# JuliaRobotics/IncrementalInference.jl

Hardware: AMD Instinct MI355X
Metric: clique-messages/sec (higher is better)
Workload: dtype f64; 1 GPU; config 2: ContinuousEuclid(2) 1000-variable odometry chain + priors every 100, N=200 particles, nested-dissection order, full up+down solveTree; variables_per_gpu=1000, particles=200, cliques=983, parallelism=single GPU

## Files before the change

include/nbp.h:

```cpp
#ifndef NBP_H
#define NBP_H

#include <stdint.h>

#ifdef __cplusplus
extern "C" {
#endif

#define NBP_MAXV 6
#define NBP_MAXF 128
#define NBP_MAXD 3
#define NBP_MAXC 4
#define NBP_MAXK 8
#define NBP_MAXN 512
#define NBP_COMP_STRIDE 13
enum nbp_dist {
  NBP_DIST_GAUSSIAN = 0,
  NBP_DIST_UNIFORM = 1,
  NBP_DIST_RAYLEIGH = 2,
  NBP_DIST_TABLE = 3
};

typedef int32_t nbp_status;
#define NBP_OK 0
// ... 326 lines not shown
  NBP_STAGE_COPIES = 3,
  NBP_STAGE_DECONV = 4,
  NBP_STAGE_COPY_POINTS = 5
};
nbp_status nbp_program_create(nbp_ctx *ctx, nbp_program **out);
nbp_status nbp_program_add_stage(nbp_program *prog, int32_t kind, const void *descs, int32_t n);
enum nbp_program_option { NBP_OPT_LAZY_BANDWIDTH = 1, NBP_OPT_GRAPH_REPLAY = 2, NBP_OPT_FUSED_UPDATES = 3,
                          NBP_OPT_ASYNC_UPLOAD = 4  };
nbp_status nbp_program_set_option(nbp_program *prog, int32_t option, int32_t value);
nbp_status nbp_program_finalize(nbp_program *prog);
nbp_status nbp_program_run(nbp_program *prog, int32_t first_stage, int32_t last_stage );
nbp_status nbp_program_reseed(nbp_program *prog, uint64_t salt);
nbp_status nbp_program_num_seeds(nbp_program *prog, int32_t *out);
nbp_status nbp_program_set_seeds(nbp_program *prog, const uint64_t *seeds, int32_t n);
nbp_status nbp_program_seed_order(nbp_program *prog, int32_t *order, int32_t n);
nbp_status nbp_program_num_stages(nbp_program *prog, int32_t *out);
nbp_status nbp_program_num_fused(nbp_program *prog, int32_t *out);
nbp_status nbp_program_num_two_stream(nbp_program *prog, int32_t *out);
nbp_status nbp_program_set_lanes(nbp_program *prog, int32_t stage, const int32_t *lane_of_descriptor, int32_t n);
typedef struct nbp_lane_part_rec {
  int32_t stage, lane, first_desc, n, wait, signals;
} nbp_lane_part_rec;
nbp_status nbp_program_lane_plan(nbp_program *prog, nbp_lane_part_rec *out, int32_t cap, int32_t *n_out);
nbp_status nbp_program_destroy(nbp_program *prog);
nbp_status nbp_program_retire(nbp_program *prog);

#define NBP_COMM_ID_BYTES 128
typedef struct nbp_comm nbp_comm;
#ifndef NBP_XFER_DEFINED
#define NBP_XFER_DEFINED
typedef struct nbp_xfer { int32_t peer; int32_t slot; } nbp_xfer;
#endif
nbp_status nbp_comm_unique_id(void *id_out );
nbp_status nbp_comm_create(nbp_ctx *ctx, int32_t world, int32_t rank, const void *id, nbp_comm **out);
nbp_status nbp_comm_destroy(nbp_comm *comm);
nbp_status nbp_comm_info(nbp_comm *comm, int32_t *nranks_out, int32_t *rank_out);
nbp_status nbp_exchange(nbp_ctx *ctx, nbp_comm *comm, const nbp_xfer *sends, int32_t n_sends, const nbp_xfer *recvs, int32_t n_recvs);

nbp_status nbp_timing_enable(nbp_ctx *ctx, int32_t on);
nbp_status nbp_timing_read(nbp_ctx *ctx, double *ms, int64_t *launches);
nbp_status nbp_timing_read_n(nbp_ctx *ctx, double *ms, int64_t *launches, int32_t n);
nbp_status nbp_diag_read(nbp_ctx *ctx, nbp_diag *out, int32_t reset);

typedef struct nbp_product_plan_req {
  int32_t N;
  int32_t n;
// ... 60 lines not shown
```

include/nbp_host.h:

```cpp
#ifndef NBP_HOST_H
#define NBP_HOST_H
#include "nbp.h"

#ifdef __cplusplus
extern "C" {
#endif

typedef struct nbp_graph nbp_graph;
typedef struct nbp_tree nbp_tree;

typedef struct nbp_solver_params {
  int32_t N;
  int32_t gibbs_iters;
  int32_t inflate_cycles;
  int32_t product_niter;
  int32_t upsolve, downsolve, limitfixeddown;
  int32_t flags;
  double spread_nh;
  double inflation;
  double null_surplus_add;
} nbp_solver_params;

enum nbp_solver_flag {
  NBP_SOLVER_STORED_MEASUREMENTS = 1,
// ... 122 lines not shown
  const nbp_solver_params *params;
  const nbp_clique_desc *clique;
  uint64_t seed;
  nbp_tree_belief *beliefs;
  nbp_tree_belief *diff_out;
  int32_t down;
  int32_t status;
} nbp_clique_request;
nbp_status nbp_clique_solve_batch(nbp_ctx *ctx, nbp_clique_request *requests, int32_t n);

typedef struct nbp_clique_ticket nbp_clique_ticket;
nbp_status nbp_clique_submit_batch(nbp_ctx *ctx, nbp_clique_request *requests, int32_t n, nbp_clique_ticket **ticket_out);
nbp_status nbp_clique_wait(nbp_clique_ticket *ticket);
nbp_status nbp_resident_write(nbp_ctx *ctx, int32_t n, const int32_t *handles, const int32_t *manifolds, const nbp_tree_belief *beliefs);
nbp_status nbp_resident_read(nbp_ctx *ctx, int32_t n, const int32_t *handles, const int32_t *manifolds, nbp_tree_belief *beliefs);
nbp_status nbp_resident_copy(nbp_ctx *ctx, int32_t n, const int32_t *src_handles, const int32_t *dst_handles, int32_t points_only);

nbp_status nbp_clique_seam_times(double *seconds_out6, int32_t mode);

int32_t nbp_tree_num_stages(const nbp_tree *t);
nbp_status nbp_tree_stage(const nbp_tree *t, int32_t s, int32_t *kind, int32_t *n, void *descs_out, int64_t cap_bytes);
nbp_status nbp_tree_stage_lanes(const nbp_tree *t, int32_t s, int32_t *lanes_out, int32_t cap);
nbp_status nbp_tree_stage_promoted(const nbp_tree *t, int32_t s, int32_t *promoted_out, int32_t cap);

#ifdef __cplusplus
}
#endif
#endif
```

incrementalinference.jl_amd/abi.py:

```python
import ctypes as C
import os

MAXV, MAXF, MAXD, MAXC, MAXN, COMP_STRIDE = 6, 128, 3, 4, 512, 13

EUCLID1, EUCLID2, EUCLID3, CIRCULAR, SE2 = 1, 2, 3, 4, 5
F_PRIOR, F_MSGPRIOR, F_LINREL, F_CIRCULAR, F_SE2, F_EUCLIDDIST, F_PASSTHROUGH = 1, 2, 3, 4, 5, 6, 7
DIST_GAUSSIAN, DIST_UNIFORM, DIST_RAYLEIGH, DIST_TABLE = 0, 1, 2, 3
STAGE_PROPOSALS, STAGE_PRODUCTS, STAGE_COPIES, STAGE_DECONV, STAGE_COPY_POINTS = 1, 2, 3, 4, 5
OPT_LAZY_BANDWIDTH = 1
OPT_GRAPH_REPLAY = 2
OPT_FUSED_UPDATES = 3

MANIFOLD_DIM = {EUCLID1: 1, EUCLID2: 2, EUCLID3: 3, CIRCULAR: 1, SE2: 3}
MANIFOLD_P = {EUCLID1: 1, EUCLID2: 2, EUCLID3: 3, CIRCULAR: 1, SE2: 6}


class ProposalDesc(C.Structure):
    _fields_ = [
        ("factor_kind", C.c_int32),
        ("manifold", C.c_int32),
        ("nvars", C.c_int32),
        ("sfidx", C.c_int32),
        ("var_slot", C.c_int32 * MAXV),
        ("out_slot", C.c_int32),
# ... 204 lines not shown
def plan_fits(reqs):
    return _plan("nbp_plan_fits", FitPlanReq, FitPlanRec, reqs)


def plan_proposals(reqs):
    return _plan("nbp_plan_proposals", ProposalPlanReq, ProposalPlanRec, reqs)


def slot_stride(N):
    return 3 * N + 8


_PKG_DIR = os.path.dirname(os.path.abspath(__file__))
LIB_PATH = os.path.join(_PKG_DIR, "csrc", "libnbp.so")

EXPORTS = [
    "nbp_arena_bytes", "nbp_slot_stride_doubles", "nbp_ctx_create", "nbp_ctx_destroy",
    "nbp_last_error", "nbp_synchronize", "nbp_arena_ptr", "nbp_stream_ptr", "nbp_ctx_particles", "nbp_ctx_slots", "nbp_ctx_device",
    "nbp_ctx_reserve_resident", "nbp_ctx_resident", "nbp_belief_write_batch_async", "nbp_belief_read_batch_begin", "nbp_belief_read_batch_end",
    "nbp_run_copies_async", "nbp_program_retire",
    "nbp_slot_write", "nbp_slot_read", "nbp_belief_write", "nbp_belief_read", "nbp_belief_write_batch", "nbp_belief_read_batch", "nbp_run_resample", "nbp_side_write", "nbp_side_read",
    "nbp_run_proposals", "nbp_run_bandwidth", "nbp_run_ppe", "nbp_kde_ppe", "nbp_run_evaluate", "nbp_kde_evaluate", "nbp_run_marginal_grid", "nbp_kde_marginal_grid", "nbp_run_evaluate_marginal", "nbp_run_mmd", "nbp_kde_mmd", "nbp_run_meancov", "nbp_kde_meancov", "nbp_run_kld", "nbp_kde_kld", "nbp_run_overlap", "nbp_kde_overlap", "nbp_run_overlap_search", "nbp_run_scene_grid", "nbp_run_credible", "nbp_kde_credible", "nbp_run_modes", "nbp_kde_modes", "nbp_run_mixture", "nbp_kde_mixture", "nbp_run_factor_likelihood", "nbp_factor_likelihood", "nbp_run_factor_mode_likelihood", "nbp_factor_mode_likelihood", "nbp_heatmap_create", "nbp_heatmap_build", "nbp_heatmap_draw", "nbp_heatmap_info", "nbp_heatmap_destroy", "nbp_heatmap_scan_eval", "nbp_heatmap_search_eval", "nbp_run_products", "nbp_run_copies", "nbp_run_deconv", "nbp_kde_bandwidth", "nbp_conv", "nbp_manifold_product",
    "nbp_program_create", "nbp_program_add_stage", "nbp_program_set_option", "nbp_program_finalize", "nbp_program_run",
    "nbp_program_reseed", "nbp_program_num_seeds", "nbp_program_set_seeds", "nbp_program_seed_order", "nbp_ctx_attach", "nbp_ctx_attached", "nbp_program_num_stages", "nbp_program_num_fused", "nbp_program_num_two_stream", "nbp_program_set_lanes", "nbp_program_lane_plan", "nbp_program_destroy",
    "nbp_timing_enable", "nbp_timing_read", "nbp_timing_read_n", "nbp_diag_read",
    "nbp_plan_products", "nbp_plan_fits", "nbp_plan_proposals", "nbp_last_plans",
    "nbp_comm_unique_id", "nbp_comm_create", "nbp_comm_destroy", "nbp_comm_info", "nbp_exchange", "nbp_math_eval",
]

_lib = None


def load_library(path=None):
    global _lib
    if _lib is not None and path is None:
        return _lib
    path = path or os.environ.get("NBP_LIB_OVERRIDE") or LIB_PATH
    if not os.path.exists(path):
        raise RuntimeError(
            f"libnbp.so not found at {path}: build it with `python __graft_entry__.py` "
            "(hipcc --offload-arch=gfx950). The product path has no CPU fallback."
        )
    try:
        import torch
    except ImportError:
        pass
    lib = C.CDLL(path)
# ... 72 lines not shown
    lib.nbp_program_add_stage.argtypes = [vp, i32, vp, i32]
    lib.nbp_program_set_option.argtypes = [vp, i32, i32]
    lib.nbp_program_finalize.argtypes = [vp]
    lib.nbp_program_run.argtypes = [vp, i32, i32]
    lib.nbp_program_reseed.argtypes = [vp, C.c_uint64]
    lib.nbp_program_num_seeds.argtypes = [vp, ip]
    lib.nbp_program_set_seeds.argtypes = [vp, C.POINTER(C.c_uint64), i32]
    lib.nbp_program_seed_order.argtypes = [vp, ip, i32]
    lib.nbp_program_num_stages.argtypes = [vp, ip]
    lib.nbp_program_destroy.argtypes = [vp]
    lib.nbp_comm_unique_id.argtypes = [vp]
    lib.nbp_comm_create.argtypes = [vp, i32, i32, vp, C.POINTER(vp)]
    lib.nbp_comm_destroy.argtypes = [vp]
    lib.nbp_comm_info.argtypes = [vp, ip, ip]
    lib.nbp_math_eval.argtypes = [vp, i32, dp, dp, dp, dp, i64]
    lib.nbp_exchange.argtypes = [vp, vp, C.POINTER(Xfer), i32, C.POINTER(Xfer), i32]
    lib.nbp_timing_enable.argtypes = [vp, i32]
    lib.nbp_timing_read.argtypes = [vp, dp, C.POINTER(i64)]
    lib.nbp_timing_read_n.argtypes = [vp, dp, C.POINTER(i64), i32]
    lib.nbp_program_num_fused.argtypes = [vp, C.POINTER(i32)]
    lib.nbp_program_num_two_stream.argtypes = [vp, C.POINTER(i32)]
    lib.nbp_program_set_lanes.argtypes = [vp, i32, ip, i32]
    lib.nbp_program_lane_plan.argtypes = [vp, C.POINTER(LanePartRec), i32, C.POINTER(i32)]
    lib.nbp_diag_read.argtypes = [vp, C.POINTER(Diag), i32]
    lib.nbp_plan_products.argtypes = [C.POINTER(ProductPlanReq), C.POINTER(ProductPlanRec), i64]
    lib.nbp_plan_fits.argtypes = [C.POINTER(FitPlanReq), C.POINTER(FitPlanRec), i64]
    lib.nbp_plan_proposals.argtypes = [C.POINTER(ProposalPlanReq), C.POINTER(ProposalPlanRec), i64]
    lib.nbp_last_plans.argtypes = [vp, C.POINTER(ProductPlanRec), C.POINTER(FitPlanRec), C.POINTER(FitPlanRec)]
    for name in EXPORTS:
        fn = getattr(lib, name)
        if fn.restype is C.c_int:
            fn.restype = C.c_int32
    if path == LIB_PATH:
        _lib = lib
    return lib
```

incrementalinference.jl_amd/backend.py:

```python
import ctypes as C
import weakref

import numpy as np

from . import abi


class NbpError(RuntimeError):
    """Hard error from libnbp (status < 0).  The Julia shim maps this to `error()`, which fails
    the clique Task and makes `monitorCSMs` tear the solve down with a CompositeException
    (reference: CliqStateMachineUtils.jl:184-246, test/testCSMMonitor.jl:51)."""


_IP, _DP = C.POINTER(C.c_int32), C.POINTER(C.c_double)


def _i32(seq):
    a = np.ascontiguousarray(seq, dtype=np.int32)
    return a, a.ctypes.data_as(_IP)


def _f64(a, shape=None):
    a = np.ascontiguousarray(a, dtype=np.float64)
    a = a if shape is None else a.reshape(shape)
# ... 662 lines not shown
        self._p = C.c_void_p()
        backend._check(lib.nbp_program_create(backend._ctx, C.byref(self._p)))
        backend._programs.add(self)
        if lazy_bandwidth:
            backend._check(lib.nbp_program_set_option(self._p, abi.OPT_LAZY_BANDWIDTH, 1))
        if not fused_updates:
            backend._check(lib.nbp_program_set_option(self._p, abi.OPT_FUSED_UPDATES, 0))
        for kind, descs in stages:
            arr, n = _as_array(descs, _STAGE_CTYPE[kind])
            backend._check(lib.nbp_program_add_stage(self._p, kind, C.cast(arr, C.c_void_p), n))
        for s, hint in (lanes or {}).items():
            arr = (C.c_int32 * max(len(hint), 1))(*[int(x) for x in hint])
            backend._check(lib.nbp_program_set_lanes(self._p, s, arr, len(hint)))
        backend._check(lib.nbp_program_finalize(self._p))
        self.n_stages = len(stages)

    def lane_plan(self):
        n = C.c_int32(0)
        self.backend._check(self.backend.lib.nbp_program_lane_plan(self._p, None, 0, C.byref(n)))
        recs = (abi.LanePartRec * max(n.value, 1))()
        self.backend._check(self.backend.lib.nbp_program_lane_plan(self._p, recs, n.value, C.byref(n)))
        return [{k: getattr(r, k) for k, _ in abi.LanePartRec._fields_} for r in recs[:n.value]]

    def num_fused(self):
        n = C.c_int32(0)
        self.backend._check(self.backend.lib.nbp_program_num_fused(self._p, C.byref(n)))
        return n.value

    def num_two_stream(self):
        n = C.c_int32(0)
        self.backend._check(self.backend.lib.nbp_program_num_two_stream(self._p, C.byref(n)))
        return n.value

    def run(self, first=0, last=-1):
        self.backend._check(self.backend.lib.nbp_program_run(self._p, first, last))

    def reseed(self, salt):
        self.backend._check(self.backend.lib.nbp_program_reseed(self._p, C.c_uint64(salt)))

    def num_seeds(self):
        n = C.c_int32(0)
        self.backend._check(self.backend.lib.nbp_program_num_seeds(self._p, C.byref(n)))
        return n.value

    def set_seeds(self, seeds):
        arr = (C.c_uint64 * len(seeds))(*[int(x) for x in seeds])
# ... 32 lines not shown
```

incrementalinference.jl_amd/csrc/nbp_api.hip:

```cpp
#include <hip/hip_runtime.h>

#include <cmath>
#include <cstdio>
#include <cstring>
#include <string>
#include <thread>
#include <vector>

#include <unordered_map>

#include <dlfcn.h>
#include <algorithm>
#include <rccl/rccl.h>

#ifndef NBP_TU
#define NBP_TU 0
#endif
#include "nbp_kernels.h"
#include "nbp_fused.h"
#include "nbp_ppe.h"
#include "nbp_query.h"
#include "nbp_stats.h"
#include "nbp_marginal.h"
#include "nbp_heatmap.h"
// ... 2578 lines not shown
  NBPCHK(stage_columns(c, {{slots, 4 * (size_t)n}, {manifolds, 4 * (size_t)n}}, d, 0));
  NBPCHK(launch_checked(c, nbp_resample_kernel, n, 256, 0, d[0], d[1], c->arena, c->N, c->S, seed));
  HIPCHK(hipStreamSynchronize(c->stream));
  return NBP_OK;
}

struct nbp_stage {
  int kind = 0, n = 0, maxfd = 0, mani = 0;
  size_t offset = 0;
  nbp_fits ent;
  bool flush_before = false;
  bool need_prep = true;
  bool fused = false, fused_second = false;
  int upd_F = 0;
  std::vector<nbp_update_desc> upd;
  size_t upd_off = 0;
  nbp_fits split_out;
  bool pipe = false;
  int pipe_split = -1, pipe_ent = 0;
  std::vector<int> moved_to;
  std::vector<int32_t> lane_hint;
  int lane_split = -1;
  int lane = 0, user = -1;
  nbp_fits bound;
  std::vector<int> waits;
  bool signals = false;
};
struct nbp_program {
  nbp_ctx *ctx = nullptr;
  std::vector<nbp_stage> stages;
  std::vector<char> blob;
  char *dev = nullptr;
  size_t dev_bytes = 0;
  bool finalized = false;
  bool lazy_bw = false;
  bool use_graph = true;
  bool use_fused = true;
  bool async_upload = false;
  int n_user_stages = 0;
  struct captured { hipGraphExec_t exec; uint64_t ws_gen; };
  std::unordered_map<uint64_t, captured> graphs;
  std::unordered_map<uint64_t, int> runs;
  size_t seed_off = 0;
  size_t seed_val_off = 0;
  int n_seeds = 0;
  std::vector<int32_t> seed_rank;
// ... 446 lines not shown
      if (n == 0 && (l || st.lane_split >= 0)) continue;
      nbp_stage pt;
      pt.kind = st.kind; pt.n = n; pt.offset = st.offset + (size_t)from * esz; pt.lane = l; pt.user = s;
      pt.maxfd = st.maxfd; pt.mani = st.mani;
      if (st.kind == NBP_STAGE_PRODUCTS && st.lane_split >= 0) {
        pt.maxfd = products_maxfd((const nbp_product_desc *)(p->blob.data() + pt.offset), n);
        pt.mani = products_uniform_manifold((const nbp_product_desc *)(p->blob.data() + pt.offset), n);
      }
      if (st.kind == NBP_STAGE_PROPOSALS && st.lane_split >= 0) pt.mani = proposals_uniform_class((const nbp_proposal_desc *)(p->blob.data() + pt.offset), n);
      const std::vector<char> &row = st.kind == NBP_STAGE_PRODUCTS ? live.dead_product[(size_t)s] : live.dead_proposal[(size_t)s];
      dead.push_back(row.empty() ? nullptr : row.data() + from);
      parts.push_back(std::move(pt));
    }
  }
  p->first_part[(size_t)p->n_user_stages] = (int)parts.size();
  {
    nbp_stage pt;
    pt.user = p->n_user_stages;
    dead.push_back(nullptr);
    parts.push_back(std::move(pt));
  }
  nbp_fits pend[2];
  std::vector<nbp_fits> ran(parts.size());
  for (int k = 0; k < (int)parts.size(); k++) {
    nbp_stage &st = parts[(size_t)k];
    const int l = st.lane, o = 1 - l;
    const char *d = p->blob.data() + st.offset;
    if (k == p->first_part[(size_t)st.user]) {
      st.bound = pend[0];
      for (const nbp_fits::fit &f : pend[1].v) st.bound.push(f.slot, f.mani);
    }
    if (st.kind == NBP_STAGE_DECONV || st.kind == NBP_STAGE_COPY_POINTS)
      stage_writes(p, st, [&](int, int32_t slot) { pend[0].drop(slot); pend[1].drop(slot); });
    if (!pend[o].empty()) {
      auto claim = [&](int32_t slot) {
        for (size_t i = 0; i < pend[o].v.size();)
          if (pend[o].v[i].slot == slot) { pend[l].v.push_back(pend[o].v[i]); pend[o].v.erase(pend[o].v.begin() + (long)i); } else i++;
      };
      stage_reads(p, st, [&](int, int32_t slot, nbp_access a) { if (a != NBP_RD_POINTS || st.kind == NBP_STAGE_PRODUCTS) claim(slot); });
      if (st.kind == NBP_STAGE_PROPOSALS || st.kind == NBP_STAGE_PRODUCTS) stage_writes(p, st, [&](int, int32_t slot) { claim(slot); });
      if (st.kind == NBP_STAGE_COPIES || st.kind == 0) {
        for (const nbp_fits::fit &f : pend[o].v) pend[l].v.push_back(f);
        pend[o].clear();
      }
    }
    st.ent = pend[l];
    auto flush_if_read = [&](nbp_access what) {
      stage_reads(p, st, [&](int, int32_t slot, nbp_access a) { st.flush_before |= a == what && pend[l].has(slot); });
      if (st.flush_before) { for (const nbp_fits::fit &f : pend[l].v) ran[(size_t)k].push(f.slot, f.mani); pend[l].clear(); }
    };
    if (st.kind == NBP_STAGE_PROPOSALS) {
      flush_if_read(NBP_RD_KDE);
      queue_fits(pend[l], (const nbp_proposal_desc *)d, st.n, dead[(size_t)k]);
    } else if (st.kind == NBP_STAGE_PRODUCTS) {
      const nbp_product_desc *qd = (const nbp_product_desc *)d;
      st.need_prep = false;
      for (int i = 0; i < st.n; i++) st.need_prep |= qd[i].nfactors > 1;
      flush_if_read(NBP_RD_POINTS);
      if (st.need_prep) {
        for (const nbp_fits::fit &f : pend[l].v) ran[(size_t)k].push(f.slot, f.mani);
        pend[l].clear();
      } else {
        for (int i = 0; i < st.n; i++) pend[l].rename(qd[i].in_slot[0], qd[i].out_slot);
        pend[l].dedup();
      }
      queue_fits(pend[l], qd, st.n, dead[(size_t)k]);
    } else if (st.kind == NBP_STAGE_DECONV || st.kind == NBP_STAGE_COPY_POINTS) {
      if (st.kind == NBP_STAGE_DECONV)
        for (int i = 0; i < st.n; i++) pend[l].push(((const nbp_proposal_desc *)d)[i].out_slot, ((const nbp_proposal_desc *)d)[i].manifold);
    } else {
      st.flush_before = true;
      for (const nbp_fits::fit &f : pend[l].v) ran[(size_t)k].push(f.slot, f.mani);
      pend[l].clear();
    }
  }
  std::vector<nbp_lane_part> sw(parts.size());
  for (int k = 0; k < (int)parts.size(); k++) {
    const nbp_stage &st = parts[(size_t)k];
    nbp_lane_part &a = sw[(size_t)k];
    a.stage = st.user;
    a.lane = st.lane;
    a.barrier = st.kind == 0 || ((st.kind == NBP_STAGE_COPIES || st.kind == NBP_STAGE_COPY_POINTS) && st.n == 0);
    stage_reads(p, st, [&](int, int32_t slot, nbp_access acc) {
      a.reads.push_back(2 * slot);
      if (acc != NBP_RD_POINTS || st.kind == NBP_STAGE_PRODUCTS) a.reads.push_back(2 * slot + 1);
      if (acc == NBP_RD_POINTS && st.kind == NBP_STAGE_PRODUCTS) a.writes.push_back(2 * slot);
    }, true);
    stage_writes(p, st, [&](int, int32_t slot) {
      a.writes.push_back(2 * slot);
      if (st.kind != NBP_STAGE_COPY_POINTS) a.writes.push_back(2 * slot + 1);
    });
    for (const nbp_fits::fit &f : ran[(size_t)k].v) { a.reads.push_back(2 * f.slot); a.writes.push_back(2 * f.slot + 1); }
    const char *d = p->blob.data() + st.offset;
    for (int i = 0; i < st.n; i++)
      if (st.kind == NBP_STAGE_PROPOSALS || st.kind == NBP_STAGE_DECONV) {
        const nbp_proposal_desc &q = ((const nbp_proposal_desc *)d)[i];
        if (q.mhidx_in >= 0) a.reads.push_back(NBP_LANE_SLOT_SIDE);
        if (q.mhidx_out >= 0) a.writes.push_back(NBP_LANE_SLOT_SIDE);
      } else if (st.kind == NBP_STAGE_PRODUCTS && ((const nbp_product_desc *)d)[i].labels_out >= 0) {
        a.writes.push_back(NBP_LANE_SLOT_SIDE);
      }
  }
  nbp_lane_sweep(sw);
  for (int k = 0; k < (int)parts.size(); k++) {
    parts[(size_t)k].waits = sw[(size_t)k].waits;
// ... 395 lines not shown
nbp_status nbp_program_num_two_stream(nbp_program *p, int32_t *out) {
  if (!p || !out) return fail(NBP_ERR_ARG, "null argument");
  int n = 0;
  for (const nbp_stage &st : p->stages) n += st.pipe ? 1 : 0;
  *out = n;
  return NBP_OK;
}

nbp_status nbp_program_lane_plan(nbp_program *p, nbp_lane_part_rec *out, int32_t cap, int32_t *n_out) {
  if (!p || !n_out || (!out && cap > 0)) return fail(NBP_ERR_ARG, "null argument");
  if (!p->finalized) return fail(NBP_ERR_ARG, "program not finalized");
  const int np = p->parts.empty() ? 0 : (int)p->parts.size() - 1;
  *n_out = np;
  for (int k = 0; k < np && k < cap; k++) {
    const nbp_stage &st = p->parts[(size_t)k];
    const nbp_stage &us = p->stages[(size_t)st.user];
    const size_t esz = st.kind == NBP_STAGE_PRODUCTS ? sizeof(nbp_product_desc) : (st.kind == NBP_STAGE_COPIES || st.kind == NBP_STAGE_COPY_POINTS ?
                       sizeof(nbp_copy_desc) : sizeof(nbp_proposal_desc));
    out[k] = {st.user, st.lane, (int32_t)((st.offset - us.offset) / esz), st.n, st.waits.empty() ? -1 : st.waits[0], st.signals ? 1 : 0};
  }
  return NBP_OK;
}

static void program_free(nbp_program *p, bool sync);
static void reap_retired(nbp_ctx *c) {
  for (size_t i = 0; i < c->retired.size();) {
    if (hipEventQuery(c->retired[i].second) == hipSuccess) {
      hipEventDestroy(c->retired[i].second);
      nbp_program *p = c->retired[i].first;
      c->retired.erase(c->retired.begin() + (long)i);
      program_free(p, false);
    } else
      i++;
  }
}
nbp_status nbp_program_retire(nbp_program *p) {
  if (!p) return NBP_OK;
  if (!p->ctx) { delete p; return NBP_OK; }
  nbp_ctx *c = p->ctx;
  hipSetDevice(c->device);
  reap_retired(c);
  hipEvent_t ev = nullptr;
  if (hipEventCreateWithFlags(&ev, hipEventDisableTiming) != hipSuccess || hipEventRecord(ev, c->stream) != hipSuccess) {
    if (ev) hipEventDestroy(ev);
    return nbp_program_destroy(p);
  }
// ... 370 lines not shown
```

incrementalinference.jl_amd/csrc/nbp_host.cpp:

```cpp
#include <algorithm>
#include <atomic>
#include <chrono>
#include <array>
#include <deque>
#include <cstdio>
#include <cstdlib>
#include <cstring>
#include <map>
#include <set>
#include <string>
#include <condition_variable>
#include <functional>
#include <mutex>
#include <thread>
#include <vector>

#include "../../include/nbp_host.h"

extern "C" nbp_status nbp_internal_fail(nbp_status code, const char *msg);
static nbp_status hfail(nbp_status c, const char *m) { return nbp_internal_fail(c, m); }

namespace {

struct HVar { int manifold; bool initialized, ismargin; };
// ... 1162 lines not shown
    for (const Clique &c : t->cl) {
      if (!(start[c.id] <= tt && tt < finish[c.id]) || !t->mine(c.id)) continue;
      const std::vector<int> &round = (down ? t->drounds : t->urounds)[c.id - 1][tt - start[c.id]];
      for (size_t lane = 0; lane < round.size(); lane++) {
        const int k = round[lane], v = (down ? t->dsched : t->usched)[c.id - 1][k];
        const bool fresh = down || !t->stored || t->uiter[c.id - 1][k] == 1;
        if (nbp_status rc = tree_update(t, c, v, down ? down_entries(t, c, v) : up_entries(t, c, v), down ? PASS_DOWN : PASS_UP, k, seed, props,
                                        prods, fresh, (int)lane))
          return rc;
      }
      plane.resize(props.size(), side.empty() ? 0 : side[c.id]);
      qlane.resize(prods.size(), side.empty() ? 0 : side[c.id]);
    }
    if (!prods.empty()) {
      add_update_stages(t->stages, props, prods);
      if (!side.empty()) {
        t->stages[t->stages.size() - 2].lane = plane;
        t->stages[t->stages.size() - 1].lane = qlane;
      }
    }
    return (nbp_status)NBP_OK;
  };
  const long round_updates = 200;
  auto stragglers = [&](bool down, int T, const std::vector<int> &start, const std::vector<int> &finish) {
    std::vector<char> side;
    if (!t->owner.empty() || T <= 0) return side;
    const int narrow_max = getenv("NBP_LANE_NARROW_MAX") ? atoi(getenv("NBP_LANE_NARROW_MAX")) : 32;
    const bool promote = down && !(getenv("NBP_LANE_NO_PROMOTE") && atoi(getenv("NBP_LANE_NO_PROMOTE")) != 0);
    const auto &rounds = down ? t->drounds : t->urounds;
    std::vector<int> count((size_t)T, 0), held((size_t)T, 0);
    for (const Clique &c : t->cl)
      for (int tt = start[c.id]; tt < finish[c.id]; tt++) count[(size_t)tt] += (int)rounds[c.id - 1][(size_t)(tt - start[c.id])].size();
    side.assign(t->cl.size() + 1, 0);
    bool any = false;
    for (const Clique &c : t->cl) {
      bool narrow = false, wide = false;
      for (int tt = start[c.id]; tt < finish[c.id]; tt++) {
        if (count[(size_t)tt] <= narrow_max) narrow = true; else wide = true;
      }
      if (!(narrow && wide)) continue;
      side[c.id] = 1;
      any = true;
      for (int tt = start[c.id]; tt < finish[c.id]; tt++) held[(size_t)tt] += (int)rounds[c.id - 1][(size_t)(tt - start[c.id])].size();
    }
    if (!any || *std::max_element(held.begin(), held.end()) > 64) side.clear();
    if (side.empty() || !promote) return side;
    std::vector<char> chain(side);
    for (const Clique &c : t->cl) {
      if (!side[c.id]) continue;
      long ahead = 0;
      for (int tt = start[c.id]; tt < T; tt++)
        if (count[(size_t)tt] > narrow_max) ahead += count[(size_t)tt];
      if ((long)(finish[c.id] - start[c.id]) * round_updates <= ahead) continue;
      for (int a = c.parent; a != 0 && !chain[a]; a = t->cl[a - 1].parent) {
        bool wide = false;
        for (int tt = start[a]; tt < finish[a]; tt++) wide |= count[(size_t)tt] > narrow_max;
        if (!wide) break;
        chain[a] = 2;
        for (int tt = start[a]; tt < finish[a]; tt++) held[(size_t)tt] += (int)rounds[a - 1][(size_t)(tt - start[a])].size();
      }
    }
    return *std::max_element(held.begin(), held.end()) > 64 ? side : chain;
  };
  if (g->sp.upsolve) {
    const size_t nc = t->cl.size();
    const std::vector<int> ids = cliques_by(height);
    std::vector<int> start(nc + 1, 0), finish(nc + 1, 0);
    int T = 0;
    for (int cid : ids) {
      int st = 0;
      for (int chd : t->cl[cid - 1].children) st = std::max(st, finish[chd]);
      start[cid] = st;
      finish[cid] = st + (int)t->urounds[cid - 1].size();
      T = std::max(T, finish[cid]);
    }
    const std::vector<char> side = stragglers(false, T, start, finish);
    for (int tt = 0; tt < T; tt++) {
      if (t->joint) {
        props.clear();
        for (const Clique &c : t->cl) {
          if (finish[c.id] != tt || c.parent == 0 || !t->mine(c.id)) continue;
          for (size_t i = 0; i < c.rel.size(); i++)
            props.push_back(deconv_op(g->sp, seed, c.id, (int)i, c.rel[i][3], c.rel[i][0], c.rel[i][1], g->vars[c.rel[i][0]].manifold,
                                      g->vars[c.rel[i][1]].manifold, {&t->B[c.id - 1], &t->main_slot}, c.Dslot[i]));
        }
// ... 16 lines not shown
  };
  cps.clear();
  if (!g->sp.downsolve) {
    for (const Clique &c : t->cl) frontals_out(c, cps);
    add_stage(t->stages, NBP_STAGE_COPIES, cps.data(), sizeof(nbp_copy_desc), (int)cps.size());
  } else {
    for (int r : t->roots) frontals_out(t->cl[r - 1], cps);
    add_stage(t->stages, NBP_STAGE_COPIES, cps.data(), sizeof(nbp_copy_desc), (int)cps.size());
    std::vector<nbp_copy_desc> final_cps;
    for (int dpt = 1; dpt <= maxd; dpt++)
      for (const Clique &c : t->cl)
        if (depth[c.id] == dpt) frontals_out(c, final_cps);
    {
      const size_t nc = t->cl.size();
      const std::vector<int> ids = cliques_by(depth);
      std::vector<int> start(nc + 1, 0), finish(nc + 1, 0);
      int T = 0;
      for (int cid : ids) {
        const Clique &c = t->cl[cid - 1];
        start[cid] = c.parent ? finish[c.parent] : 0;
        finish[cid] = start[cid] + (int)t->drounds[cid - 1].size();
        T = std::max(T, finish[cid]);
      }
      const std::vector<char> side = stragglers(true, T, start, finish);
      for (int tt = 0; tt <= T; tt++) {
        std::map<int, int> rnd;
        int nrounds = 0;
        for (int cid : ids) {
          const Clique &c = t->cl[cid - 1];
          if (start[cid] != tt || !c.parent) continue;
          auto it = rnd.find(c.parent);
          rnd[cid] = it == rnd.end() ? 0 : it->second + 1;
          nrounds = std::max(nrounds, rnd[cid] + 1);
        }
        for (int r = 0; r < nrounds; r++) {
          std::vector<Edge> edges;
          for (const Clique &c : t->cl) {
            auto it = rnd.find(c.id);
            if (it == rnd.end() || it->second != r || t->own(c.id) == t->own(c.parent)) continue;
            for (int s : c.seps)
              edges.push_back({t->own(c.parent), t->mine(c.parent) ? t->B[c.parent - 1].at(s) : -1, t->own(c.id),
                               t->mine(c.id) ? t->B[c.id - 1].at(s) : -1});
          }
          rank_exchange(t, edges);
          cps.clear();
          std::vector<int32_t> clane;
          for (const Clique &c : t->cl) {
// ... 1146 lines not shown
  if (mode >= 1) g_seam_sync.store(mode == 2);
  return NBP_OK;
}

int32_t nbp_tree_num_stages(const nbp_tree *t) { return t ? (int32_t)t->stages.size() : 0; }
nbp_status nbp_tree_stage(const nbp_tree *t, int32_t s, int32_t *kind, int32_t *n, void *out, int64_t cap) {
  if (!t || s < 0 || s >= (int)t->stages.size()) return hfail(NBP_ERR_RANGE, "stage index");
  return stage_out(t->stages[s], kind, n, out, cap);
}
nbp_status nbp_tree_stage_lanes(const nbp_tree *t, int32_t s, int32_t *lanes_out, int32_t cap) {
  if (!t || s < 0 || s >= (int)t->stages.size()) return hfail(NBP_ERR_RANGE, "stage index");
  if (!lanes_out && cap > 0) return hfail(NBP_ERR_ARG, "null argument");
  const Stage &st = t->stages[s];
  for (int i = 0; i < st.n && i < cap; i++) lanes_out[i] = !st.lane.empty() && st.lane[(size_t)i] == 1;
  return NBP_OK;
}
nbp_status nbp_tree_stage_promoted(const nbp_tree *t, int32_t s, int32_t *promoted_out, int32_t cap) {
  if (!t || s < 0 || s >= (int)t->stages.size()) return hfail(NBP_ERR_RANGE, "stage index");
  if (!promoted_out && cap > 0) return hfail(NBP_ERR_ARG, "null argument");
  const Stage &st = t->stages[s];
  for (int i = 0; i < st.n && i < cap; i++) promoted_out[i] = !st.lane.empty() && st.lane[(size_t)i] == 2;
  return NBP_OK;
}

}
```

incrementalinference.jl_amd/native_host.py:

```python
import ctypes as C

import numpy as np

from . import abi

i32, i64, f64 = C.c_int32, C.c_int64, C.c_double


SOLVER_STORED_MEASUREMENTS, SOLVER_MSG_LIKELIHOODS = 1, 2


class SolverParamsC(C.Structure):
    _fields_ = [("N", i32), ("gibbs_iters", i32), ("inflate_cycles", i32), ("product_niter", i32), ("upsolve", i32),
                ("downsolve", i32), ("limitfixeddown", i32), ("flags", i32), ("spread_nh", f64), ("inflation", f64),
                ("null_surplus_add", f64)]


class FactorSpec(C.Structure):
    _fields_ = [("factor_kind", i32), ("nvars", i32), ("vars", i32 * abi.MAXV), ("ncomp", i32), ("has_multihypo", i32),
                ("partial_mask", i32), ("multihypo", f64 * abi.MAXV), ("nullhypo", f64), ("inflation", f64),
                ("comp", (f64 * abi.COMP_STRIDE) * abi.MAXC)]


class CliqueInfo(C.Structure):
# ... 12 lines not shown
class TreeBeliefC(C.Structure):
    _fields_ = [("pts", C.POINTER(f64)), ("bw", C.POINTER(f64)), ("ipc", C.POINTER(f64)), ("n_pts", i32), ("handle", i32)]


class CliqueDescC(C.Structure):
    _fields_ = [("clique_id", i32), ("nvars", i32), ("nfrontals", i32), ("nseparators", i32),
                ("manifold", C.POINTER(i32)), ("ismargin", C.POINTER(i32)), ("nfactors", i32), ("factors", C.POINTER(FactorSpec)),
                ("n_direct_frtl_msg", i32), ("n_msgskip", i32), ("n_itervar", i32), ("n_direct_prior_msg", i32),
                ("direct_frtl_msg", C.POINTER(i32)), ("msgskip", C.POINTER(i32)), ("itervar", C.POINTER(i32)),
                ("direct_prior_msg", C.POINTER(i32)), ("nmsgs", i32), ("msg_var", C.POINTER(i32)),
                ("msg_belief", C.POINTER(TreeBeliefC)), ("factor_density", C.POINTER(TreeBeliefC)),
                ("factor_meas_kde", C.POINTER(TreeBeliefC)), ("n_diff", i32), ("reserved_", i32),
                ("diff_a", C.POINTER(i32)), ("diff_b", C.POINTER(i32)), ("diff_kind", C.POINTER(i32))]


CLIQ_UPSOLVED, CLIQ_DOWNSOLVED = 3, 5
CLIQ_NULL, CLIQ_MARGINALIZED, CLIQ_UPRECYCLED = 0, 4, 6

HOST_EXPORTS = ["nbp_graph_create", "nbp_graph_destroy", "nbp_graph_add_variable", "nbp_graph_add_factor",
                "nbp_graph_set_variable_flags", "nbp_graph_num_variables", "nbp_graph_num_factors",
                "nbp_graph_order_nested_dissection", "nbp_graph_init_plan", "nbp_graph_init_num_variables", "nbp_graph_init_variables",
                "nbp_graph_init_num_stages", "nbp_graph_init_stage", "nbp_graph_init_compile", "nbp_tree_build", "nbp_tree_destroy", "nbp_tree_num_cliques",
                "nbp_tree_clique", "nbp_tree_clique_idlists", "nbp_tree_max_schedule", "nbp_tree_plan_slots", "nbp_tree_main_slots", "nbp_tree_compile", "nbp_tree_schedule",
                "nbp_tree_get_stats", "nbp_tree_num_stages", "nbp_tree_stage", "nbp_tree_stage_lanes", "nbp_tree_stage_promoted", "nbp_clique_slots", "nbp_clique_upsolve", "nbp_clique_upsolve_joint", "nbp_clique_downsolve", "nbp_clique_solve_batch", "nbp_clique_seam_times",
                "nbp_clique_submit_batch", "nbp_clique_wait", "nbp_resident_write", "nbp_resident_read", "nbp_resident_copy",
                "nbp_tree_partition", "nbp_tree_set_owner", "nbp_tree_num_segments", "nbp_tree_segment",
                "nbp_tree_run_sharded", "nbp_tree_run_sharded_cb",
                "nbp_graph_num_densities", "nbp_graph_density_factors", "nbp_graph_init_density_slot0", "nbp_tree_density_slot0",
                "nbp_tree_set_clique_status", "nbp_tree_clique_status", "nbp_tree_recycle", "nbp_tree_cliques_recycled"]

_declared = False


def _lib():
    global _declared
    lib = abi.load_library()
    if not _declared:
        vp, ip = C.c_void_p, C.POINTER(i32)
        lib.nbp_graph_create.argtypes = [C.POINTER(SolverParamsC), C.POINTER(vp)]
        lib.nbp_graph_destroy.argtypes = [vp]
        lib.nbp_graph_add_variable.argtypes = [vp, i32]
        lib.nbp_graph_add_factor.argtypes = [vp, C.POINTER(FactorSpec)]
        lib.nbp_graph_set_variable_flags.argtypes = [vp, i32, i32, i32]
        lib.nbp_graph_num_variables.argtypes = [vp]
        lib.nbp_graph_num_factors.argtypes = [vp]
        lib.nbp_graph_order_nested_dissection.argtypes = [vp, ip]
        lib.nbp_graph_init_plan.argtypes = [vp, C.c_uint64]
# ... 1 lines not shown
        lib.nbp_graph_num_densities.argtypes = [vp]
        lib.nbp_graph_density_factors.argtypes = [vp, ip]
        lib.nbp_graph_init_density_slot0.argtypes = [vp]
        lib.nbp_tree_density_slot0.argtypes = [vp]
        lib.nbp_graph_init_variables.argtypes = [vp, ip]
        lib.nbp_graph_init_num_stages.argtypes = [vp]
        lib.nbp_graph_init_stage.argtypes = [vp, i32, ip, ip, vp, i64]
        lib.nbp_graph_init_compile.argtypes = [vp, vp, C.POINTER(vp)]
        lib.nbp_tree_build.argtypes = [vp, ip, i32, C.POINTER(vp)]
        lib.nbp_tree_destroy.argtypes = [vp]
        lib.nbp_tree_num_cliques.argtypes = [vp]
        lib.nbp_tree_clique.argtypes = [vp, i32, C.POINTER(CliqueInfo), ip, ip, ip, ip, ip, ip]
        lib.nbp_tree_max_schedule.argtypes = [vp]
        lib.nbp_tree_clique_idlists.argtypes = [vp, i32, ip, ip, ip, ip, ip]
        lib.nbp_tree_plan_slots.argtypes = [vp, i32]
        lib.nbp_tree_main_slots.argtypes = [vp, ip, ip]
        lib.nbp_tree_compile.argtypes = [vp, vp, C.c_uint64, C.POINTER(vp)]
        lib.nbp_tree_schedule.argtypes = [vp, C.c_uint64]
        lib.nbp_tree_get_stats.argtypes = [vp, C.POINTER(TreeStats)]
        lib.nbp_tree_num_stages.argtypes = [vp]
        lib.nbp_tree_stage.argtypes = [vp, i32, ip, ip, vp, i64]
        lib.nbp_tree_stage_lanes.argtypes = [vp, i32, ip, i32]
        lib.nbp_tree_stage_promoted.argtypes = [vp, i32, ip, i32]
        lib.nbp_tree_partition.argtypes = [vp, i32, ip]
        lib.nbp_tree_set_owner.argtypes = [vp, ip, i32]
        lib.nbp_tree_num_segments.argtypes = [vp]
        lib.nbp_tree_segment.argtypes = [vp, i32, ip, ip, ip, ip, ip, C.POINTER(Xfer), C.POINTER(Xfer), i32]
        lib.nbp_tree_run_sharded.argtypes = [vp, vp, vp, vp]
        lib.nbp_tree_run_sharded_cb.argtypes = [vp, vp, XCHG_FN, vp]
        lib.nbp_tree_set_clique_status.argtypes = [vp, i32, i32]
        lib.nbp_tree_clique_status.argtypes = [vp, i32, ip, ip, ip]
        lib.nbp_tree_recycle.argtypes = [vp, vp, i32]
        lib.nbp_tree_cliques_recycled.argtypes = [vp, ip]
        lib.nbp_clique_slots.argtypes = [C.POINTER(CliqueDescC)]
        for fn in (lib.nbp_clique_upsolve, lib.nbp_clique_downsolve):
            fn.argtypes = [vp, C.POINTER(SolverParamsC), C.POINTER(CliqueDescC), C.c_uint64, C.POINTER(TreeBeliefC), ip]
        lib.nbp_clique_upsolve_joint.argtypes = [vp, C.POINTER(SolverParamsC), C.POINTER(CliqueDescC), C.c_uint64, C.POINTER(TreeBeliefC),
                                                 C.POINTER(TreeBeliefC), ip]
        lib.nbp_clique_solve_batch.argtypes = [vp, C.POINTER(CliqueRequestC), i32]
        lib.nbp_clique_seam_times.argtypes = [C.POINTER(C.c_double), i32]
        for n in HOST_EXPORTS:
            getattr(lib, n).restype = i32
        _declared = True
    return lib


# ... 398 lines not shown
        return _stages_of(lambda s, kind, n, buf, cap: self.lib.nbp_tree_stage(self._t, s, kind, n, buf, cap),
                          self.lib.nbp_tree_num_stages(self._t))

    def stage_lanes(self):
        out = []
        for s in range(self.lib.nbp_tree_num_stages(self._t)):
            kind, n = C.c_int32(0), C.c_int32(0)
            _check(self.lib.nbp_tree_stage(self._t, s, C.byref(kind), C.byref(n), None, 0))
            arr = (i32 * max(n.value, 1))()
            _check(self.lib.nbp_tree_stage_lanes(self._t, s, arr, n.value))
            out.append(list(arr[:n.value]))
        return out

    def stage_promoted(self):
        out = []
        for s in range(self.lib.nbp_tree_num_stages(self._t)):
            kind, n = C.c_int32(0), C.c_int32(0)
            _check(self.lib.nbp_tree_stage(self._t, s, C.byref(kind), C.byref(n), None, 0))
            arr = (i32 * max(n.value, 1))()
            _check(self.lib.nbp_tree_stage_promoted(self._t, s, arr, n.value))
            out.append(list(arr[:n.value]))
        return out

    def close(self):
        if self._t:
            self.lib.nbp_tree_destroy(self._t)
            self._t = C.c_void_p()

    def __del__(self):
        try:
            self.close()
        except Exception:
            pass


def clique_seam_times(mode=0):
    out = (C.c_double * 6)()
    _check(_lib().nbp_clique_seam_times(out, mode))
    return dict(zip(("planning_s", "beliefs_in_s", "assembly_s", "launches_s", "beliefs_out_s", "calls"), list(out)))
```

Measured before the change: 144,400 messages/s.

## Descend side-lane assignment to subtrees below straggler cliques in downsolve

Extends the two-lane downsolve scheduler so that cliques below a straggler clique that needs lane 1 are also placed on the side lane, marked with lane code 3, unless this would push per-round held updates past 64. It also inserts flush-only copy parts before trailing copy stages so that pending bandwidth fits on both lanes are flushed without acting as a full barrier. The goal is to let long straggler chains and their subtrees overlap with wide main-lane work instead of serializing at barriers. The cost is more complex lane and fit bookkeeping and a risk of extra cross-lane waits. Introspection APIs are added for descended cliques and per-part fits.

```diff
diff --git a/include/nbp.h b/include/nbp.h
--- a/include/nbp.h
+++ b/include/nbp.h
@@ -372,6 +372,7 @@
   int32_t stage, lane, first_desc, n, wait, signals;
 } nbp_lane_part_rec;
 nbp_status nbp_program_lane_plan(nbp_program *prog, nbp_lane_part_rec *out, int32_t cap, int32_t *n_out);
+nbp_status nbp_program_lane_part_fits(nbp_program *prog, int32_t part, int32_t *slots_out, int32_t cap, int32_t *n_out);
 nbp_status nbp_program_destroy(nbp_program *prog);
 nbp_status nbp_program_retire(nbp_program *prog);
 
diff --git a/include/nbp_host.h b/include/nbp_host.h
--- a/include/nbp_host.h
+++ b/include/nbp_host.h
@@ -168,6 +168,7 @@
 nbp_status nbp_tree_stage(const nbp_tree *t, int32_t s, int32_t *kind, int32_t *n, void *descs_out, int64_t cap_bytes);
 nbp_status nbp_tree_stage_lanes(const nbp_tree *t, int32_t s, int32_t *lanes_out, int32_t cap);
 nbp_status nbp_tree_stage_promoted(const nbp_tree *t, int32_t s, int32_t *promoted_out, int32_t cap);
+nbp_status nbp_tree_stage_descended(const nbp_tree *t, int32_t s, int32_t *descended_out, int32_t cap);
 
 #ifdef __cplusplus
 }
diff --git a/incrementalinference.jl_amd/abi.py b/incrementalinference.jl_amd/abi.py
--- a/incrementalinference.jl_amd/abi.py
+++ b/incrementalinference.jl_amd/abi.py
@@ -250,7 +250,7 @@
     "nbp_slot_write", "nbp_slot_read", "nbp_belief_write", "nbp_belief_read", "nbp_belief_write_batch", "nbp_belief_read_batch", "nbp_run_resample", "nbp_side_write", "nbp_side_read",
     "nbp_run_proposals", "nbp_run_bandwidth", "nbp_run_ppe", "nbp_kde_ppe", "nbp_run_evaluate", "nbp_kde_evaluate", "nbp_run_marginal_grid", "nbp_kde_marginal_grid", "nbp_run_evaluate_marginal", "nbp_run_mmd", "nbp_kde_mmd", "nbp_run_meancov", "nbp_kde_meancov", "nbp_run_kld", "nbp_kde_kld", "nbp_run_overlap", "nbp_kde_overlap", "nbp_run_overlap_search", "nbp_run_scene_grid", "nbp_run_credible", "nbp_kde_credible", "nbp_run_modes", "nbp_kde_modes", "nbp_run_mixture", "nbp_kde_mixture", "nbp_run_factor_likelihood", "nbp_factor_likelihood", "nbp_run_factor_mode_likelihood", "nbp_factor_mode_likelihood", "nbp_heatmap_create", "nbp_heatmap_build", "nbp_heatmap_draw", "nbp_heatmap_info", "nbp_heatmap_destroy", "nbp_heatmap_scan_eval", "nbp_heatmap_search_eval", "nbp_run_products", "nbp_run_copies", "nbp_run_deconv", "nbp_kde_bandwidth", "nbp_conv", "nbp_manifold_product",
     "nbp_program_create", "nbp_program_add_stage", "nbp_program_set_option", "nbp_program_finalize", "nbp_program_run",
-    "nbp_program_reseed", "nbp_program_num_seeds", "nbp_program_set_seeds", "nbp_program_seed_order", "nbp_ctx_attach", "nbp_ctx_attached", "nbp_program_num_stages", "nbp_program_num_fused", "nbp_program_num_two_stream", "nbp_program_set_lanes", "nbp_program_lane_plan", "nbp_program_destroy",
+    "nbp_program_reseed", "nbp_program_num_seeds", "nbp_program_set_seeds", "nbp_program_seed_order", "nbp_ctx_attach", "nbp_ctx_attached", "nbp_program_num_stages", "nbp_program_num_fused", "nbp_program_num_two_stream", "nbp_program_set_lanes", "nbp_program_lane_plan", "nbp_program_lane_part_fits", "nbp_program_destroy",
     "nbp_timing_enable", "nbp_timing_read", "nbp_timing_read_n", "nbp_diag_read",
     "nbp_plan_products", "nbp_plan_fits", "nbp_plan_proposals", "nbp_last_plans",
     "nbp_comm_unique_id", "nbp_comm_create", "nbp_comm_destroy", "nbp_comm_info", "nbp_exchange", "nbp_math_eval",
@@ -369,6 +369,7 @@
     lib.nbp_program_num_two_stream.argtypes = [vp, C.POINTER(i32)]
     lib.nbp_program_set_lanes.argtypes = [vp, i32, ip, i32]
     lib.nbp_program_lane_plan.argtypes = [vp, C.POINTER(LanePartRec), i32, C.POINTER(i32)]
+    lib.nbp_program_lane_part_fits.argtypes = [vp, i32, ip, i32, C.POINTER(i32)]
     lib.nbp_diag_read.argtypes = [vp, C.POINTER(Diag), i32]
     lib.nbp_plan_products.argtypes = [C.POINTER(ProductPlanReq), C.POINTER(ProductPlanRec), i64]
     lib.nbp_plan_fits.argtypes = [C.POINTER(FitPlanReq), C.POINTER(FitPlanRec), i64]
diff --git a/incrementalinference.jl_amd/backend.py b/incrementalinference.jl_amd/backend.py
--- a/incrementalinference.jl_amd/backend.py
+++ b/incrementalinference.jl_amd/backend.py
@@ -708,6 +708,13 @@
         self.backend._check(self.backend.lib.nbp_program_lane_plan(self._p, recs, n.value, C.byref(n)))
         return [{k: getattr(r, k) for k, _ in abi.LanePartRec._fields_} for r in recs[:n.value]]
 
+    def lane_part_fits(self, part):
+        n = C.c_int32(0)
+        self.backend._check(self.backend.lib.nbp_program_lane_part_fits(self._p, part, None, 0, C.byref(n)))
+        slots = (C.c_int32 * max(n.value, 1))()
+        self.backend._check(self.backend.lib.nbp_program_lane_part_fits(self._p, part, slots, n.value, C.byref(n)))
+        return list(slots[:n.value])
+
     def num_fused(self):
         n = C.c_int32(0)
         self.backend._check(self.backend.lib.nbp_program_num_fused(self._p, C.byref(n)))
diff --git a/incrementalinference.jl_amd/csrc/nbp_api.hip b/incrementalinference.jl_amd/csrc/nbp_api.hip
--- a/incrementalinference.jl_amd/csrc/nbp_api.hip
+++ b/incrementalinference.jl_amd/csrc/nbp_api.hip
@@ -2624,6 +2624,7 @@
   std::vector<int32_t> lane_hint;
   int lane_split = -1;
   int lane = 0, user = -1;
+  bool flush_only = false;
   nbp_fits bound;
   std::vector<int> waits;
   bool signals = false;
@@ -3116,7 +3117,20 @@
   }
   nbp_fits pend[2];
   std::vector<nbp_fits> ran(parts.size());
+  int tail = p->n_user_stages;
+  while (tail > 0 && p->stages[(size_t)tail - 1].kind == NBP_STAGE_COPIES && p->stages[(size_t)tail - 1].lane_split < 0) tail--;
   for (int k = 0; k < (int)parts.size(); k++) {
+    if (tail < p->n_user_stages && k == p->first_part[(size_t)tail] && !parts[(size_t)k].flush_only && !pend[1].empty()) {
+      for (int l = 1; l >= 0; l--) {
+        if (pend[l].empty()) continue;
+        nbp_stage pt;
+        pt.kind = NBP_STAGE_COPIES; pt.offset = p->stages[(size_t)tail].offset; pt.lane = l; pt.user = tail; pt.flush_only = true;
+        parts.insert(parts.begin() + k, std::move(pt));
+        dead.insert(dead.begin() + k, nullptr);
+        ran.insert(ran.begin() + k, nbp_fits());
+        for (int s = tail + 1; s <= p->n_user_stages; s++) p->first_part[(size_t)s]++;
+      }
+    }
     nbp_stage &st = parts[(size_t)k];
     const int l = st.lane, o = 1 - l;
     const char *d = p->blob.data() + st.offset;
@@ -3133,7 +3147,7 @@
       };
       stage_reads(p, st, [&](int, int32_t slot, nbp_access a) { if (a != NBP_RD_POINTS || st.kind == NBP_STAGE_PRODUCTS) claim(slot); });
       if (st.kind == NBP_STAGE_PROPOSALS || st.kind == NBP_STAGE_PRODUCTS) stage_writes(p, st, [&](int, int32_t slot) { claim(slot); });
-      if (st.kind == NBP_STAGE_COPIES || st.kind == 0) {
+      if ((st.kind == NBP_STAGE_COPIES && !st.flush_only) || st.kind == 0) {
         for (const nbp_fits::fit &f : pend[o].v) pend[l].v.push_back(f);
         pend[o].clear();
       }
@@ -3174,7 +3188,7 @@
     nbp_lane_part &a = sw[(size_t)k];
     a.stage = st.user;
     a.lane = st.lane;
-    a.barrier = st.kind == 0 || ((st.kind == NBP_STAGE_COPIES || st.kind == NBP_STAGE_COPY_POINTS) && st.n == 0);
+    a.barrier = st.kind == 0 || ((st.kind == NBP_STAGE_COPIES || st.kind == NBP_STAGE_COPY_POINTS) && st.n == 0 && !st.flush_only);
     stage_reads(p, st, [&](int, int32_t slot, nbp_access acc) {
       a.reads.push_back(2 * slot);
       if (acc != NBP_RD_POINTS || st.kind == NBP_STAGE_PRODUCTS) a.reads.push_back(2 * slot + 1);
@@ -3616,6 +3630,17 @@
   return NBP_OK;
 }
 
+nbp_status nbp_program_lane_part_fits(nbp_program *p, int32_t part, int32_t *slots_out, int32_t cap, int32_t *n_out) {
+  if (!p || !n_out || (!slots_out && cap > 0)) return fail(NBP_ERR_ARG, "null argument");
+  if (!p->finalized) return fail(NBP_ERR_ARG, "program not finalized");
+  if (part < 0 || part + 1 >= (int)p->parts.size()) return fail(NBP_ERR_RANGE, "lane_part_fits: no such part");
+  const nbp_stage &st = p->parts[(size_t)part];
+  const bool runs = st.flush_before || (st.kind == NBP_STAGE_PRODUCTS && st.need_prep);
+  *n_out = runs ? st.ent.size() : 0;
+  for (int i = 0; i < *n_out && i < cap; i++) slots_out[i] = st.ent.v[(size_t)i].slot;
+  return NBP_OK;
+}
+
 static void program_free(nbp_program *p, bool sync);
 static void reap_retired(nbp_ctx *c) {
   for (size_t i = 0; i < c->retired.size();) {
diff --git a/incrementalinference.jl_amd/csrc/nbp_host.cpp b/incrementalinference.jl_amd/csrc/nbp_host.cpp
--- a/incrementalinference.jl_amd/csrc/nbp_host.cpp
+++ b/incrementalinference.jl_amd/csrc/nbp_host.cpp
@@ -1208,8 +1208,11 @@
     return (nbp_status)NBP_OK;
   };
   const long round_updates = 200;
+  bool promotion_capped = false;
+  std::vector<char> needs_lane1;
   auto stragglers = [&](bool down, int T, const std::vector<int> &start, const std::vector<int> &finish) {
     std::vector<char> side;
+    promotion_capped = false;
     if (!t->owner.empty() || T <= 0) return side;
     const int narrow_max = getenv("NBP_LANE_NARROW_MAX") ? atoi(getenv("NBP_LANE_NARROW_MAX")) : 32;
     const bool promote = down && !(getenv("NBP_LANE_NO_PROMOTE") && atoi(getenv("NBP_LANE_NO_PROMOTE")) != 0);
@@ -1230,7 +1233,8 @@
       for (int tt = start[c.id]; tt < finish[c.id]; tt++) held[(size_t)tt] += (int)rounds[c.id - 1][(size_t)(tt - start[c.id])].size();
     }
     if (!any || *std::max_element(held.begin(), held.end()) > 64) side.clear();
-    if (side.empty() || !promote) return side;
+    needs_lane1.assign(side.size(), 0);
+    if (side.empty() || !down) return side;
     std::vector<char> chain(side);
     for (const Clique &c : t->cl) {
       if (!side[c.id]) continue;
@@ -1238,6 +1242,8 @@
       for (int tt = start[c.id]; tt < T; tt++)
         if (count[(size_t)tt] > narrow_max) ahead += count[(size_t)tt];
       if ((long)(finish[c.id] - start[c.id]) * round_updates <= ahead) continue;
+      needs_lane1[c.id] = 1;
+      if (!promote) continue;
       for (int a = c.parent; a != 0 && !chain[a]; a = t->cl[a - 1].parent) {
         bool wide = false;
         for (int tt = start[a]; tt < finish[a]; tt++) wide |= count[(size_t)tt] > narrow_max;
@@ -1246,7 +1252,24 @@
         for (int tt = start[a]; tt < finish[a]; tt++) held[(size_t)tt] += (int)rounds[a - 1][(size_t)(tt - start[a])].size();
       }
     }
-    return *std::max_element(held.begin(), held.end()) > 64 ? side : chain;
+    promotion_capped = promote && *std::max_element(held.begin(), held.end()) > 64;
+    return promotion_capped ? side : chain;
+  };
+  const bool descend = !(getenv("NBP_LANE_NO_DESCEND") && atoi(getenv("NBP_LANE_NO_DESCEND")) != 0);
+  auto descendants = [&](int T, const std::vector<int> &start, const std::vector<int> &finish, const std::vector<char> &side) {
+    if (side.empty() || !descend || promotion_capped) return side;
+    std::vector<char> all(side);
+    std::vector<int> held((size_t)T, 0);
+    for (const Clique &c : t->cl) {
+      if (!side[c.id]) {
+        bool below = false;
+        for (int a = c.parent; a != 0 && !below; a = t->cl[a - 1].parent) below = side[a] == 1 && needs_lane1[a];
+        if (!below) continue;
+        all[c.id] = 3;
+      }
+      for (int tt = start[c.id]; tt < finish[c.id]; tt++) held[(size_t)tt] += (int)t->drounds[c.id - 1][(size_t)(tt - start[c.id])].size();
+    }
+    return *std::max_element(held.begin(), held.end()) > 64 ? side : all;
   };
   if (g->sp.upsolve) {
     const size_t nc = t->cl.size();
@@ -1309,7 +1332,7 @@
         finish[cid] = start[cid] + (int)t->drounds[cid - 1].size();
         T = std::max(T, finish[cid]);
       }
-      const std::vector<char> side = stragglers(true, T, start, finish);
+      const std::vector<char> side = descendants(T, start, finish, stragglers(true, T, start, finish));
       for (int tt = 0; tt <= T; tt++) {
         std::map<int, int> rnd;
         int nrounds = 0;
@@ -2502,5 +2525,12 @@
   for (int i = 0; i < st.n && i < cap; i++) promoted_out[i] = !st.lane.empty() && st.lane[(size_t)i] == 2;
   return NBP_OK;
 }
-
-}
+nbp_status nbp_tree_stage_descended(const nbp_tree *t, int32_t s, int32_t *descended_out, int32_t cap) {
+  if (!t || s < 0 || s >= (int)t->stages.size()) return hfail(NBP_ERR_RANGE, "stage index");
+  if (!descended_out && cap > 0) return hfail(NBP_ERR_ARG, "null argument");
+  const Stage &st = t->stages[(size_t)s];
+  for (int i = 0; i < st.n && i < cap; i++) descended_out[i] = !st.lane.empty() && st.lane[(size_t)i] == 3;
+  return NBP_OK;
+}
+
+}
diff --git a/incrementalinference.jl_amd/native_host.py b/incrementalinference.jl_amd/native_host.py
--- a/incrementalinference.jl_amd/native_host.py
+++ b/incrementalinference.jl_amd/native_host.py
@@ -58,7 +58,7 @@
                 "nbp_graph_order_nested_dissection", "nbp_graph_init_plan", "nbp_graph_init_num_variables", "nbp_graph_init_variables",
                 "nbp_graph_init_num_stages", "nbp_graph_init_stage", "nbp_graph_init_compile", "nbp_tree_build", "nbp_tree_destroy", "nbp_tree_num_cliques",
                 "nbp_tree_clique", "nbp_tree_clique_idlists", "nbp_tree_max_schedule", "nbp_tree_plan_slots", "nbp_tree_main_slots", "nbp_tree_compile", "nbp_tree_schedule",
-                "nbp_tree_get_stats", "nbp_tree_num_stages", "nbp_tree_stage", "nbp_tree_stage_lanes", "nbp_tree_stage_promoted", "nbp_clique_slots", "nbp_clique_upsolve", "nbp_clique_upsolve_joint", "nbp_clique_downsolve", "nbp_clique_solve_batch", "nbp_clique_seam_times",
+                "nbp_tree_get_stats", "nbp_tree_num_stages", "nbp_tree_stage", "nbp_tree_stage_lanes", "nbp_tree_stage_promoted", "nbp_tree_stage_descended", "nbp_clique_slots", "nbp_clique_upsolve", "nbp_clique_upsolve_joint", "nbp_clique_downsolve", "nbp_clique_solve_batch", "nbp_clique_seam_times",
                 "nbp_clique_submit_batch", "nbp_clique_wait", "nbp_resident_write", "nbp_resident_read", "nbp_resident_copy",
                 "nbp_tree_partition", "nbp_tree_set_owner", "nbp_tree_num_segments", "nbp_tree_segment",
                 "nbp_tree_run_sharded", "nbp_tree_run_sharded_cb",
@@ -106,6 +106,7 @@
         lib.nbp_tree_stage.argtypes = [vp, i32, ip, ip, vp, i64]
         lib.nbp_tree_stage_lanes.argtypes = [vp, i32, ip, i32]
         lib.nbp_tree_stage_promoted.argtypes = [vp, i32, ip, i32]
+        lib.nbp_tree_stage_descended.argtypes = [vp, i32, ip, i32]
         lib.nbp_tree_partition.argtypes = [vp, i32, ip]
         lib.nbp_tree_set_owner.argtypes = [vp, ip, i32]
         lib.nbp_tree_num_segments.argtypes = [vp]
@@ -550,6 +551,16 @@
             out.append(list(arr[:n.value]))
         return out
 
+    def stage_descended(self):
+        out = []
+        for s in range(self.lib.nbp_tree_num_stages(self._t)):
+            kind, n = C.c_int32(0), C.c_int32(0)
+            _check(self.lib.nbp_tree_stage(self._t, s, C.byref(kind), C.byref(n), None, 0))
+            arr = (i32 * max(n.value, 1))()
+            _check(self.lib.nbp_tree_stage_descended(self._t, s, arr, n.value))
+            out.append(list(arr[:n.value]))
+        return out
+
     def close(self):
         if self._t:
             self.lib.nbp_tree_destroy(self._t)
```

New measurement: 145,300 messages/s (median of 6 runs). Within noise of the previous version (+0.6%).
